# unanan/UNet_Nested4Tiny_Objects_Keypoints

Hardware: AMD Instinct MI355X
Metric: images/sec (train step) UNet++ L=4 256x256 (higher is better)
Workload: dtype f32

## Files before the change

### unet_nested4tiny_objects_keypoints_amd/csrc/gemm_wino.hip

```cpp
#include <cstdlib>
#include <utility>

#include "bn_fused.h"
#include "common.h"
#include "gemm_units.h"
#include "lds_asm.h"
#include "wino_experiments.h"

namespace unetpp {
namespace {

typedef float f32x2 __attribute__((ext_vector_type(2)));
typedef unsigned u32x4v __attribute__((vector_size(16)));
constexpr unsigned kOutOfRange = 0x80000000u;
typedef const __attribute__((address_space(1))) void* gptr_t;
typedef __attribute__((address_space(3))) void* lptr_t;

__device__ __forceinline__ void wino_input_transform(const float (&dd)[16], float (&V)[16]) {
  float t[4][4];
#pragma unroll
  for (int j = 0; j < 4; ++j) {
    t[0][j] = dd[0 + j] - dd[8 + j];
    t[1][j] = dd[4 + j] + dd[8 + j];
    t[2][j] = dd[8 + j] - dd[4 + j];
    t[3][j] = dd[4 + j] - dd[12 + j];
  }
#pragma unroll
  for (int i = 0; i < 4; ++i) {
    V[4 * i + 0] = t[i][0] - t[i][2];
    V[4 * i + 1] = t[i][1] + t[i][2];
    V[4 * i + 2] = t[i][2] - t[i][1];
    V[4 * i + 3] = t[i][1] - t[i][3];
  }
}

__device__ __forceinline__ void wino_input_transform_pk(const f32x2_t (&dd)[8], float (&V)[16]) {
  f32x2_t t[8];
#pragma unroll
  for (int p = 0; p < 2; ++p) {
    t[0 + p] = pk_sub(dd[0 + p], dd[4 + p]);
    t[2 + p] = pk_add(dd[2 + p], dd[4 + p]);
    t[4 + p] = pk_sub(dd[4 + p], dd[2 + p]);
    t[6 + p] = pk_sub(dd[2 + p], dd[6 + p]);
  }
#pragma unroll
  for (int i = 0; i < 4; ++i) {
    const f32x2_t va = pk_sub_add_x(t[2 * i], t[2 * i + 1]);
    const f32x2_t vb = pk_cross_sub(t[2 * i], t[2 * i + 1]);
    V[4 * i + 0] = va[0];
    V[4 * i + 1] = va[1];
    V[4 * i + 2] = vb[0];
    V[4 * i + 3] = vb[1];
  }
}

constexpr int WKC = 8;
constexpr int WNC = 32;
constexpr int WP = 10;
constexpr int WIMG = 4096;

#define WINO_FENCE() __builtin_amdgcn_sched_barrier(0)

template <int LOG2TW, int NH, int MODE, bool BNF = false>
__global__ __launch_bounds__(kThreads, 2) void gemm_wino_kernel(const FastArgs a) {
  constexpr bool LEAN = MODE != 0, FOLD = MODE == 2;
  constexpr int TW = 1 << LOG2TW, TH = kBlockPixels >> LOG2TW;
  constexpr int HWp = TW + 2, HHp = TH + 2;
  constexpr int NPIX = HWp * HHp;
  constexpr int TXN = TW / 2;
  constexpr int IN_FLOATS = 4096;
  constexpr int IN_ITEMS = (NPIX * 2 + kThreads - 1) / kThreads;
  constexpr int W_ITEMS = WIMG / 4 / kThreads;
  static_assert(IN_ITEMS == 3 && W_ITEMS == 4, "the staging lambdas' default ranges");
  static_assert(kMaxHaloPixels * WP <= IN_FLOATS, "input patch does not fit");
  static_assert(((IN_ITEMS * kThreads - 1) >> 1) * WP + 8 <= IN_FLOATS, "staging items past the patch must stay inside the buffer");
  constexpr int BUF = IN_FLOATS + WIMG;
  __shared__ __attribute__((aligned(16))) float smem[2 * BUF];
  float* in_tile = smem;
  float* w_tile = smem + IN_FLOATS;
  constexpr int RUN0 = 4 * WNC * 2;
  __shared__ float stat_lds[BNF ? RUN0 + kBnFusedMaxCols * 2 : RUN0];
  constexpr int kBiasCols = 512;
  __shared__ __attribute__((aligned(16))) float bias_lds[kBiasCols];

  const unetpp_gemm_desc& d = a.d;
  const int tid = threadIdx.x;
  const int wave = __builtin_amdgcn_readfirstlane(tid >> 6), lane = tid & 63, t16 = lane & 15, g = lane >> 4;

  const UnitRange ur = my_contiguous_unit_range(a.total_blocks);
  for (int i = tid; i < kBiasCols; i += kThreads)
    bias_lds[i] = (a.d.bias != nullptr && i < a.Ncols) ? a.d.bias[i] : 0.f;
  constexpr bool bn_fused = BNF;
  if constexpr (BNF) {
    for (int i = tid; i < kBnFusedMaxCols * 2; i += kThreads) stat_lds[RUN0 + i] = 0.f;
  }
  if (ur.count == 0) {
    if constexpr (BNF) {
      __syncthreads();
      bn_rows_store<kThreads>(a.d.stats_partial, a.Ncols, stat_lds + RUN0);
    }
    return;
  }
  const int n_units = __builtin_amdgcn_readfirstlane(static_cast<int>(ur.count));

  const int my_tile = 16 * wave + t16;
  const int a_base = ((2 * (my_tile / TXN)) * HWp + 2 * (my_tile % TXN)) * WP + 2 * g;
  const int b_base = (g * 16 + t16) * 2;

  f32x4 acc[16][NH];
#pragma unroll
  for (int xi = 0; xi < 16; ++xi)
#pragma unroll
    for (int nh = 0; nh < NH; ++nh) acc[xi][nh] = f32x4{0.f, 0.f, 0.f, 0.f};

  f32x4 reg_in[IN_ITEMS];
  unsigned voff[IN_ITEMS];
  unsigned in_mask = 0;
  int pf_cnt = 0;
  int p_unit = 0;
  int p_s = 0, p_c0 = 0, p_chunk = 0;
  int p_n = 0, p_ty0 = 0, p_tx0 = 0;
  const float* p_wimg = nullptr;
  const int cc = (tid & 1) << 2;
  const float* v_ptr = nullptr;
  const float* v_scale = nullptr;
  const float* v_shift = nullptr;
  int v_clen = 0;
  bool v_relu = false;
  int v_bytes = 0, v_pitch = 0, v_origin = 0;
  int pix[IN_ITEMS];
  auto cache_view = [&]() {
    const unetpp_view& V = d.in[p_s];
    v_clen = V.c_len;
    if constexpr (LEAN) {
      v_ptr = V.ptr;
      v_bytes = d.N * V.Hs * V.Ws * V.C * 4;
      v_pitch = V.C * 4;
      v_origin = V.c_off * 4;
      if constexpr (FOLD) {
        v_scale = V.scale;
        v_shift = V.shift;
        v_relu = V.relu != 0;
      }
    } else {
      v_ptr = V.ptr;
      v_scale = V.scale;
      v_shift = V.shift;
      v_relu = V.relu != 0;
    }
  };

  auto step_unit = [&](UnitGeom& u) {
    if (++u.group < a.n_groups) return;
    u.group = 0;
    ++u.patch;
    u.tx0 += TW;
    if (u.tx0 < a.tiles_x * TW) return;
    u.tx0 = 0;
    u.ty0 += TH;
    if (u.ty0 < a.tiles_y * TH) return;
    u.ty0 = 0;
    ++u.n;
  };
  UnitGeom p_ug = decode_unit<LOG2TW>(a, ur.first);
  p_ug.n = __builtin_amdgcn_readfirstlane(p_ug.n);
  p_ug.ty0 = __builtin_amdgcn_readfirstlane(p_ug.ty0);
  p_ug.tx0 = __builtin_amdgcn_readfirstlane(p_ug.tx0);
  p_ug.group = __builtin_amdgcn_readfirstlane(p_ug.group);
  p_ug.patch = __builtin_amdgcn_readfirstlane(static_cast<int>(p_ug.patch));
  UnitGeom c_ug = p_ug;

  long p_patch = -1;
  auto prefetch_unit = [&]() -> bool {
    const UnitGeom& ug = p_ug;
    p_wimg = d.weight_image + static_cast<long>(ug.group) * a.n_chunks * WIMG;
    if (ug.patch == p_patch) return true;
    p_patch = ug.patch;
    p_n = ug.n;
    p_ty0 = ug.ty0;
    p_tx0 = ug.tx0;
    if constexpr (LEAN) {
      const int row0 = p_n * d.H;
#pragma unroll
      for (int q = 0; q < IN_ITEMS; ++q) {
        const int it = tid + q * kThreads;
        const int hp = it >> 1;
        const int hy = hp / HWp, hx = hp - hy * HWp;
        const int y = p_ty0 + hy - 1, x = p_tx0 + hx - 1;
        const bool in_patch = ((q + 1) * kThreads <= NPIX * 2) ? true : (it < NPIX * 2);
        const bool inside = in_patch & (static_cast<unsigned>(y) < static_cast<unsigned>(d.H)) &
                            (static_cast<unsigned>(x) < static_cast<unsigned>(d.W));
        const int linear = (row0 + y) * d.W + x;
        pix[q] = inside ? linear : -1;
      }
      return false;
    }
    in_mask = 0;
#pragma unroll
    for (int q = 0; q < IN_ITEMS; ++q) {
      const int it = tid + q * kThreads;
      const int hp = it >> 1;
      const int hy = hp / HWp, hx = hp - hy * HWp;
      const int y = p_ty0 + hy - 1, x = p_tx0 + hx - 1;
      if ((it < NPIX * 2) && y >= 0 && y < d.H && x >= 0 && x < d.W) in_mask |= 1u << q;
    }
    return false;
  };
  auto view_offsets = [&](const unetpp_view& V) {
    if constexpr (LEAN) {
#pragma unroll
      for (int q = 0; q < IN_ITEMS; ++q)
        voff[q] = static_cast<unsigned>(pix[q] * v_pitch + v_origin + cc * 4) |
                  (static_cast<unsigned>(pix[q] >> 31) & kOutOfRange);
      return;
    }
#pragma unroll
    for (int q = 0; q < IN_ITEMS; ++q) {
      const int hp = min((tid + q * kThreads) >> 1, NPIX - 1);
      const int hy = hp / HWp, hx = hp - hy * HWp;
      const int yy = min(max(p_ty0 + hy - 1, 0), d.H - 1), xx = min(max(p_tx0 + hx - 1, 0), d.W - 1);
      voff[q] = view_pixel_offset32(V, p_n, yy, xx);
    }
  };
  auto advance = [&]() {
    if (p_chunk + 1 < a.n_chunks) {
      ++p_chunk;
      p_c0 += WKC;
      if (p_c0 >= v_clen) {
        ++p_s;
        p_c0 = 0;
        cache_view();
        view_offsets(d.in[p_s]);
      }
    } else if (p_unit + 1 < n_units) {
      ++p_unit;
      p_chunk = 0;
      p_c0 = 0;
      const bool same_view = p_s == 0;
      if (!same_view) {
        p_s = 0;
        cache_view();
      }
      step_unit(p_ug);
      if (!prefetch_unit() || !same_view) view_offsets(d.in[0]);
    }
  };
  f32x4 co_sc = {1.f, 1.f, 1.f, 1.f}, co_sh = {0.f, 0.f, 0.f, 0.f};
  float co_floor = 0.f;
  auto load_coeffs = [&]() {
    if constexpr (!FOLD) return;
    co_floor = v_relu ? 0.f : -__builtin_inff();
    if (v_scale != nullptr) {
      co_sc = *reinterpret_cast<const f32x4*>(v_scale + p_c0 + cc);
      co_sh = *reinterpret_cast<const f32x4*>(v_shift + p_c0 + cc);
    } else {
      co_sc = f32x4{1.f, 1.f, 1.f, 1.f};
      co_sh = f32x4{0.f, 0.f, 0.f, 0.f};
    }
  };
  auto load_inputs = [&]() {
    if constexpr (LEAN) {
      const __amdgpu_buffer_rsrc_t v_rsrc =
          __builtin_amdgcn_make_buffer_rsrc(const_cast<float*>(v_ptr), 0, v_bytes, 0x00020000);
#pragma unroll
      for (int q = 0; q < IN_ITEMS; ++q) {
        const u32x4v v = __builtin_amdgcn_raw_buffer_load_b128(v_rsrc, static_cast<int>(voff[q]), p_c0 * 4, 0);
        reg_in[q] = __builtin_bit_cast(f32x4, v);
      }
      return;
    }
    pf_cnt = min(WKC, v_clen - p_c0);
#pragma unroll
    for (int q = 0; q < IN_ITEMS; ++q) {
      const unsigned off = voff[q] + static_cast<unsigned>(p_c0 + (cc < pf_cnt ? cc : 0));
      reg_in[q] = *reinterpret_cast<const f32x4*>(v_ptr + off);
    }
  };
  auto dma_source = [&]() { return p_wimg + static_cast<long>(p_chunk) * WIMG; };
  auto dma_weights = [&](float* w_dst, const float* wp, int q0 = 0, int q1 = 4) {
#pragma unroll
    for (int q = q0; q < q1; ++q)
      __builtin_amdgcn_global_load_lds((gptr_t)(wp + (tid + q * kThreads) * 4),
                                       (lptr_t)(w_dst + (q * kThreads + wave * 64) * 4), 16, 0, 0);
  };
  auto store_chunk = [&](float* in_dst, int q0 = 0, int q1 = 3) {
    if constexpr (LEAN) {
#pragma unroll
      for (int q = q0; q < q1; ++q) {
        const int it = tid + q * kThreads;
        f32x4 v = reg_in[q];
        if constexpr (FOLD) {
          const unsigned inside = ~static_cast<unsigned>(pix[q] >> 31);
#pragma unroll
          for (int e = 0; e < 4; ++e)
            v[e] = __builtin_bit_cast(float, __builtin_bit_cast(unsigned, floor_keep_nan(fmaf(v[e], co_sc[e], co_sh[e]), co_floor)) & inside);
        }
        *reinterpret_cast<f32x2*>(&in_dst[(it >> 1) * WP + cc]) = f32x2{v[0], v[1]};
        *reinterpret_cast<f32x2*>(&in_dst[(it >> 1) * WP + cc + 2]) = f32x2{v[2], v[3]};
      }
      return;
    }
    const bool affine = v_scale != nullptr;
    f32x4 sc = {1.f, 1.f, 1.f, 1.f}, sh = {0.f, 0.f, 0.f, 0.f};
    if (affine) {
      const int ch = p_c0 + (cc < pf_cnt ? cc : 0);
      sc = *reinterpret_cast<const f32x4*>(v_scale + ch);
      sh = *reinterpret_cast<const f32x4*>(v_shift + ch);
    }
#pragma unroll
    for (int q = 0; q < IN_ITEMS; ++q) {
      const int it = tid + q * kThreads;
      const bool keep = ((in_mask >> q) & 1u) && cc < pf_cnt;
      f32x4 v = reg_in[q];
      if (affine) {
#pragma unroll
        for (int e = 0; e < 4; ++e) v[e] = fmaf(v[e], sc[e], sh[e]);
      }
      if (v_relu) {
#pragma unroll
        for (int e = 0; e < 4; ++e) v[e] = relu_keep_nan(v[e]);
      }
#pragma unroll
      for (int e = 0; e < 4; ++e) v[e] = keep ? v[e] : 0.f;
      if (it < NPIX * 2) {
        *reinterpret_cast<f32x2*>(&in_dst[(it >> 1) * WP + cc]) = f32x2{v[0], v[1]};
        *reinterpret_cast<f32x2*>(&in_dst[(it >> 1) * WP + cc + 2]) = f32x2{v[2], v[3]};
      }
    }
  };

  auto epilogue = [&]() {
    const UnitGeom& ug = c_ug;
    const TileCols tc = decode_tile(a, ug.group);
    const unetpp_view& O = d.out[tc.ov];
    const bool interior = (ug.ty0 + TH <= d.H) && (ug.tx0 + TW <= d.W);
    const unsigned rs = static_cast<unsigned>(O.sy) * O.Ws * O.C, cs = static_cast<unsigned>(O.sx) * O.C;
    const unsigned tile_base = view_pixel_offset32(O, ug.n, ug.ty0, ug.tx0) + tc.nt * WNC;
    float* obase = O.ptr + tile_base;
    const float* gbase = O.gate != nullptr ? O.gate + tile_base : nullptr;
    const bool vec_out = ((O.C | O.c_off | tc.n_cnt) & 3) == 0 && (reinterpret_cast<uintptr_t>(O.ptr) & 15) == 0 &&
                         (O.gate == nullptr || (reinterpret_cast<uintptr_t>(O.gate) & 15) == 0);
    const bool want_stats = d.stats_partial != nullptr;
    const float floor_v = O.relu ? 0.f : -__builtin_inff();
    float s1[NH][4], s2[NH][4];
#pragma unroll
    for (int nh = 0; nh < NH; ++nh)
#pragma unroll
      for (int rr = 0; rr < 4; ++rr) s1[nh][rr] = s2[nh][rr] = 0.f;
    if (d.bias != nullptr && tc.n0 + WNC <= kBiasCols) {
#pragma unroll
      for (int nh = 0; nh < NH; ++nh) acc[5][nh] += *reinterpret_cast<const f32x4*>(&bias_lds[tc.n0 + 16 * nh + 4 * g]);
    } else if (d.bias != nullptr) {
#pragma unroll
      for (int nh = 0; nh < NH; ++nh)
#pragma unroll
        for (int rr = 0; rr < 4; ++rr) {
          const int col = 16 * nh + 4 * g + rr;
          acc[5][nh][rr] += col < tc.n_cnt ? d.bias[tc.n0 + col] : 0.f;
        }
    }
    const unsigned ty2 = 2 * (my_tile / TXN), tx2 = 2 * (my_tile % TXN);
    auto out_row = [&](int ap, int nh, int rr, float (&y)[2]) {
      float tb[4];
#pragma unroll
      for (int b = 0; b < 4; ++b)
        tb[b] = (ap == 0) ? (acc[b][nh][rr] + acc[4 + b][nh][rr]) + acc[8 + b][nh][rr]
                          : (acc[4 + b][nh][rr] - acc[8 + b][nh][rr]) - acc[12 + b][nh][rr];
      y[0] = floor_keep_nan((tb[0] + tb[1]) + tb[2], floor_v);
      y[1] = floor_keep_nan((tb[1] - tb[2]) - tb[3], floor_v);
    };
    if (interior && vec_out && tc.n_cnt == 16 * NH) {
      const bool has_gate = gbase != nullptr, acc_out = O.accumulate != 0;
      const unsigned lane_off = ty2 * rs + tx2 * cs + 4 * g;
#pragma unroll
      for (int ap = 0; ap < 2; ++ap) {
        unsigned off[2][NH];
        f32x4 gt[2][NH], old[2][NH];
#pragma unroll
        for (int bp = 0; bp < 2; ++bp)
#pragma unroll
          for (int nh = 0; nh < NH; ++nh) off[bp][nh] = lane_off + ap * rs + bp * cs + 16 * nh;
        if (has_gate) {
#pragma unroll
          for (int bp = 0; bp < 2; ++bp)
#pragma unroll
            for (int nh = 0; nh < NH; ++nh) gt[bp][nh] = *reinterpret_cast<const f32x4*>(gbase + off[bp][nh]);
        }
        if (acc_out) {
#pragma unroll
          for (int bp = 0; bp < 2; ++bp)
#pragma unroll
            for (int nh = 0; nh < NH; ++nh) old[bp][nh] = *reinterpret_cast<const f32x4*>(obase + off[bp][nh]);
        }
        f32x4 yv[2][NH];
#pragma unroll
        for (int nh = 0; nh < NH; ++nh) {
          f32x2 y[2][2];
#pragma unroll
          for (int cp = 0; cp < 2; ++cp) {
            f32x2 tb[4];
#pragma unroll
            for (int b = 0; b < 4; ++b) {
              const f32x2 m0 = cp ? acc[b][nh].hi : acc[b][nh].lo, m1 = cp ? acc[4 + b][nh].hi : acc[4 + b][nh].lo;
              const f32x2 m2 = cp ? acc[8 + b][nh].hi : acc[8 + b][nh].lo, m3 = cp ? acc[12 + b][nh].hi : acc[12 + b][nh].lo;
              tb[b] = (ap == 0) ? (m0 + m1) + m2 : (m1 - m2) - m3;
            }
            const f32x2 t0 = (tb[0] + tb[1]) + tb[2], t1 = (tb[1] - tb[2]) - tb[3];
            y[0][cp] = f32x2{floor_keep_nan(t0.x, floor_v), floor_keep_nan(t0.y, floor_v)};
            y[1][cp] = f32x2{floor_keep_nan(t1.x, floor_v), floor_keep_nan(t1.y, floor_v)};
          }
          yv[0][nh] = f32x4{y[0][0].x, y[0][0].y, y[0][1].x, y[0][1].y};
          yv[1][nh] = f32x4{y[1][0].x, y[1][0].y, y[1][1].x, y[1][1].y};
          if (want_stats) {
#pragma unroll
            for (int rr = 0; rr < 4; ++rr) {
              const float y0 = yv[0][nh][rr], y1 = yv[1][nh][rr];
              s1[nh][rr] += y0 + y1;
              s2[nh][rr] = fmaf(y0, y0, fmaf(y1, y1, s2[nh][rr]));
            }
          }
        }
        if (!has_gate && !acc_out) {
#pragma unroll
          for (int bp = 0; bp < 2; ++bp)
#pragma unroll
            for (int nh = 0; nh < NH; ++nh) {
              if constexpr (wino_exp::kNoOutStore) asm volatile("" ::"v"(yv[bp][nh]), "v"(off[bp][nh]));
              else *reinterpret_cast<f32x4*>(obase + off[bp][nh]) = yv[bp][nh];
            }
          continue;
        }
#pragma unroll
        for (int bp = 0; bp < 2; ++bp)
#pragma unroll
          for (int nh = 0; nh < NH; ++nh) {
            f32x4 v = yv[bp][nh];
            if (has_gate && !O.gate_sum) {
#pragma unroll
              for (int e = 0; e < 4; ++e) v[e] = (gt[bp][nh][e] > 0.f) ? v[e] : 0.f;
            }
            if (acc_out) {
#pragma unroll
              for (int e = 0; e < 4; ++e) v[e] += old[bp][nh][e];
            }
            if (has_gate && O.gate_sum) {
#pragma unroll
              for (int e = 0; e < 4; ++e) v[e] = (gt[bp][nh][e] > 0.f) ? v[e] : 0.f;
            }
            *reinterpret_cast<f32x4*>(obase + off[bp][nh]) = v;
          }
      }
    } else {
#pragma unroll
      for (int ap = 0; ap < 2; ++ap) {
        const unsigned py = ty2 + ap;
#pragma unroll
        for (int nh = 0; nh < NH; ++nh)
#pragma unroll
          for (int rr = 0; rr < 4; ++rr) {
            float y[2];
            out_row(ap, nh, rr, y);
            const int col = 16 * nh + 4 * g + rr;
#pragma unroll
            for (int bp = 0; bp < 2; ++bp) {
              float v = y[bp];
              if ((col < tc.n_cnt) && (ug.ty0 + py < d.H) && (ug.tx0 + tx2 + bp < d.W)) {
                s1[nh][rr] += v;
                s2[nh][rr] = fmaf(v, v, s2[nh][rr]);
                const unsigned off = py * rs + (tx2 + bp) * cs + col;
                if (gbase != nullptr && !O.gate_sum) v = (gbase[off] > 0.f) ? v : 0.f;
                if (O.accumulate) v += obase[off];
                if (gbase != nullptr && O.gate_sum) v = (gbase[off] > 0.f) ? v : 0.f;
                obase[off] = v;
              }
            }
          }
      }
    }
#pragma unroll
    for (int xi = 0; xi < 16; ++xi)
#pragma unroll
      for (int nh = 0; nh < NH; ++nh) acc[xi][nh] = f32x4{0.f, 0.f, 0.f, 0.f};
    if (want_stats) {
#pragma unroll
      for (int nh = 0; nh < NH; ++nh)
#pragma unroll
        for (int rr = 0; rr < 4; ++rr) {
          s1[nh][rr] = row16_sum(s1[nh][rr]);
          s2[nh][rr] = row16_sum(s2[nh][rr]);
          if (t16 == 0) {
            stat_lds[(wave * WNC + 16 * nh + 4 * g + rr) * 2 + 0] = s1[nh][rr];
            stat_lds[(wave * WNC + 16 * nh + 4 * g + rr) * 2 + 1] = s2[nh][rr];
          }
        }
    }
  };
  auto flush_stats = [&]() {
    if (d.stats_partial == nullptr || tid >= 16 * NH) return;
    const UnitGeom& ug = c_ug;
    const TileCols tc = decode_tile(a, ug.group);
    if (tid >= tc.n_cnt) return;
    float t1 = 0.f, t2 = 0.f;
#pragma unroll
    for (int w = 0; w < 4; ++w) {
      t1 += stat_lds[(w * WNC + tid) * 2 + 0];
      t2 += stat_lds[(w * WNC + tid) * 2 + 1];
    }
    if constexpr (bn_fused) {
      stat_lds[RUN0 + (tc.n0 + tid) * 2 + 0] += t1;
      stat_lds[RUN0 + (tc.n0 + tid) * 2 + 1] += t2;
      return;
    }
    float* dst = d.stats_partial + (ug.patch * a.Ncols + tc.n0 + tid) * 2;
    dst[0] = t1;
    dst[1] = t2;
  };

  cache_view();
  prefetch_unit();
  view_offsets(d.in[0]);
  load_coeffs();
  load_inputs();
  dma_weights(w_tile, dma_source());
  store_chunk(in_tile);
  advance();
  load_coeffs();
  load_inputs();
  asm volatile("s_waitcnt vmcnt(%0)" ::"n"(IN_ITEMS) : "memory");
  __syncthreads();

  int c_chunk = 0, c_unit = 0;
  int cur = 0;
  while (true) {
    const unsigned in_b = lds_offset(in_tile) + a_base * 4, w_b = lds_offset(w_tile) + b_base * 4;
    float dd[16], ddn[16], V[16];
    f32x2_t dp[8], dpn[8];
    unsigned row_b[4];
#pragma unroll
    for (int i = 0; i < 4; ++i) row_b[i] = in_b + i * HWp * WP * 4;
    f32x4 us[2][2];
    if constexpr (LEAN) {
      static_for<8>([&](auto ic) {
        constexpr int e = decltype(ic)::v, j = 2 * (e & 1);
        lds_read2_b32<j * WP, (j + 1) * WP>(dp[e], row_b[e >> 1]);
      });
    } else {
      static_for<16>([&](auto ic) {
        constexpr int e = decltype(ic)::v;
        lds_read_b32<((e / 4) * HWp + (e % 4)) * WP * 4>(dd[e], in_b);
      });
    }
    lds_read2st64_b64<0, 1>(us[0][0], w_b);
    lds_read2st64_b64<2, 3>(us[0][1], w_b);

    float* other = smem + (cur ^ 1) * BUF;
    if constexpr (!LEAN) {
      __builtin_amdgcn_s_setprio(3);
      store_chunk(other);
      dma_weights(other + IN_FLOATS, dma_source());
      advance();
      load_inputs();
    }
    auto staging_piece = [&](auto gc) {
      constexpr int g = decltype(gc)::v;
      if constexpr (!LEAN) return;
      if constexpr (wino_exp::kNoStaging) {
        if constexpr (g == 2) advance();
        return;
      }
      if constexpr (g == 0 && !wino_exp::kNoStore) store_chunk(other);
      if constexpr (g == 0 && !wino_exp::kNoDma) dma_weights(other + IN_FLOATS, dma_source());
      if constexpr (g == 1) {
        advance();
        load_coeffs();
      }
      if constexpr (g == 2 && !wino_exp::kNoLoads) load_inputs();
    };

    __builtin_amdgcn_s_setprio(2);
    if constexpr (LEAN) {
      lds_wait8x2(dp);
      lds_wait(us[0][0], us[0][1]);
      wino_input_transform_pk(dp, V);
    } else {
      lds_wait16(dd);
      lds_wait(us[0][0], us[0][1]);
      wino_input_transform(dd, V);
    }
    static_for<8>([&](auto gc) {
      constexpr int g = decltype(gc)::v, cs = g & 1, ns = cs ^ 1;
      if constexpr (g + 1 < 8) {
        lds_read2st64_b64<4 * (g + 1), 4 * (g + 1) + 1>(us[ns][0], w_b);
        lds_read2st64_b64<4 * (g + 1) + 2, 4 * (g + 1) + 3>(us[ns][1], w_b);
      }
      if constexpr (g == 0) {
        if constexpr (LEAN) {
          static_for<8>([&](auto ic) {
            constexpr int e = decltype(ic)::v, j = 2 * (e & 1);
            lds_read2_b32<j * WP + 1, (j + 1) * WP + 1>(dpn[e], row_b[e >> 1]);
          });
        } else {
          static_for<16>([&](auto ic) {
            constexpr int e = decltype(ic)::v;
            lds_read_b32<(((e / 4) * HWp + (e % 4)) * WP + 1) * 4>(ddn[e], in_b);
          });
        }
      }
      WINO_FENCE();
#pragma unroll
      for (int q = 0; q < 4; ++q) {
        const int xi = (4 * g + q) & 15;
        const f32x4 up = us[cs][q >> 1];
        acc[xi][0] = __builtin_amdgcn_mfma_f32_16x16x4f32(up[(q & 1) * 2], V[xi], acc[xi][0], 0, 0, 0);
        if (NH == 2)
          acc[xi][NH - 1] = __builtin_amdgcn_mfma_f32_16x16x4f32(up[(q & 1) * 2 + 1], V[xi], acc[xi][NH - 1], 0, 0, 0);
      }
      staging_piece(gc);
      WINO_FENCE();
      if constexpr (g == 0) {
        if constexpr (LEAN) lds_wait8x2(dpn);
        else lds_wait16(ddn);
      }
      if constexpr (g + 1 < 8) lds_wait(us[ns][0], us[ns][1]);
      if constexpr (g == 3) {
        if constexpr (LEAN) wino_input_transform_pk(dpn, V);
        else wino_input_transform(ddn, V);
      }
    });
    __builtin_amdgcn_s_setprio(0);
    if constexpr (!wino_exp::kNoBarrier) {
      if (wino_exp::kLaxWait && c_chunk == 0 && c_unit > 0)
        asm volatile("s_waitcnt vmcnt(%0) lgkmcnt(0)" ::"n"(IN_ITEMS + 4 + 4 * NH) : "memory");
      else
      asm volatile("s_waitcnt vmcnt(%0) lgkmcnt(0)" ::"n"(IN_ITEMS) : "memory");
      __builtin_amdgcn_s_barrier();
      asm volatile("" ::: "memory");
    }
    if (c_chunk + 1 == a.n_chunks) {
#pragma unroll
      for (int q = 0; q < IN_ITEMS; ++q) asm volatile("" : "+v"(reg_in[q]));
      if constexpr (wino_exp::kNoEpilogue) {
#pragma unroll
        for (int xi = 0; xi < 16; ++xi)
#pragma unroll
          for (int nh = 0; nh < NH; ++nh) {
            asm volatile("" : "+v"(acc[xi][nh]));
            acc[xi][nh] = f32x4{0.f, 0.f, 0.f, 0.f};
          }
      } else {
        epilogue();
      }
      if (d.stats_partial != nullptr) {
        __syncthreads();
        flush_stats();
      }
      step_unit(c_ug);
      c_chunk = 0;
      if (++c_unit == n_units) break;
    } else {
      ++c_chunk;
    }
    cur ^= 1;
    in_tile = smem + cur * BUF;
    w_tile = in_tile + IN_FLOATS;
  }
  if constexpr (BNF) {
    __syncthreads();
    bn_rows_store<kThreads>(d.stats_partial, a.Ncols, stat_lds + RUN0);
  }
}

}

bool wino_applies(const unetpp_gemm_desc* d) {
  return d != nullptr && d->taps == 9 && (d->flags & (UNETPP_GEMM_DIRECT | UNETPP_GEMM_BF16)) == 0;
}

void gemm_wino_plan(const unetpp_gemm_desc* d, GemmSel& s) {
  s.kernel = GEMM_WINO;
  s.label = "gemm_wino_kernel";
  long workers = (2L * s.cus) & ~7L;
#ifdef UNETPP_WINO_EXP
  if (opt_value(OPT_WINO_ONE_PER_CU, 0) == 1) workers = s.cus & ~7L;
#endif
  if (workers < 8) workers = 8;
  if (workers > kBnFusedRows) workers = kBnFusedRows;
  s.grid_x = static_cast<unsigned>(s.fa.total_blocks <= workers ? s.fa.total_blocks : workers);
  bool narrow = true;
  for (int i = 0; i < d->n_out; ++i) narrow = narrow && d->out[i].c_len <= 16;
  bool lean = opt_value(OPT_WINO_NO_LEAN, 0) == 0, fold = false;
  for (int i = 0; i < d->n_in; ++i) {
    const unetpp_view& v = d->in[i];
    lean = lean && (v.c_len & 7) == 0 && v.Hs == d->H && v.Ws == d->W && v.sy == 1 && v.sx == 1 && v.oy == 0 &&
           v.ox == 0 && static_cast<long>(d->N) * v.Hs * v.Ws * v.C * 4 <= 0x7fffffffL;
    fold = fold || v.scale != nullptr || v.relu != 0;
  }
  s.narrow = narrow ? 1 : 0;
  s.mode = !lean ? 0 : (fold ? 2 : 1);
  s.fa.bn_in_kernel = (s.mode != 0 && bn_rows_per_workgroup(d, s.fa.Ncols)) ? 1 : 0;
  s.bn_rows = s.fa.bn_in_kernel ? s.grid_x : 0;
}

int launch_gemm_wino(const unetpp_gemm_desc*, const GemmSel& s, hipStream_t st) {
  const FastArgs& a = s.fa;
  const int mode = s.mode;
  const bool narrow = s.narrow != 0;
  const dim3 grid(s.grid_x), block(kThreads);
#define UNETPP_LAUNCH_WINO_M(L, NHV)                                                                    \
  do {                                                                                                  \
    if (mode == 0) hipLaunchKernelGGL((gemm_wino_kernel<L, NHV, 0>), grid, block, 0, st, a);            \
    else if (a.bn_in_kernel && mode == 1) hipLaunchKernelGGL((gemm_wino_kernel<L, NHV, 1, true>), grid, block, 0, st, a); \
    else if (a.bn_in_kernel) hipLaunchKernelGGL((gemm_wino_kernel<L, NHV, 2, true>), grid, block, 0, st, a);             \
    else if (mode == 1) hipLaunchKernelGGL((gemm_wino_kernel<L, NHV, 1>), grid, block, 0, st, a);       \
    else hipLaunchKernelGGL((gemm_wino_kernel<L, NHV, 2>), grid, block, 0, st, a);                      \
  } while (0)
#define UNETPP_LAUNCH_WINO(L)                 \
  do {                                        \
    if (narrow) UNETPP_LAUNCH_WINO_M(L, 1);   \
    else UNETPP_LAUNCH_WINO_M(L, 2);          \
  } while (0)
  if (a.log2tw == 5) UNETPP_LAUNCH_WINO(5);
  else if (a.log2tw == 4) UNETPP_LAUNCH_WINO(4);
  else UNETPP_LAUNCH_WINO(3);
#undef UNETPP_LAUNCH_WINO
#undef UNETPP_LAUNCH_WINO_M
  return launch_status();
}

}
```

### unet_nested4tiny_objects_keypoints_amd/csrc/lds_asm.h

```cpp
#pragma once
#include <utility>

#include "common.h"

namespace unetpp {

template <int I>
struct IC {
  static constexpr int v = I;
};
template <class F, int... I>
__device__ __forceinline__ void static_for_impl(F&& f, std::integer_sequence<int, I...>) {
  (f(IC<I>{}), ...);
}
template <int N, class F>
__device__ __forceinline__ void static_for(F&& f) {
  static_for_impl(f, std::make_integer_sequence<int, N>{});
}
__device__ __forceinline__ unsigned lds_offset(const float* p) {
  return static_cast<unsigned>(reinterpret_cast<uintptr_t>(p));
}
template <int OFF>
__device__ __forceinline__ void lds_read_b32(float& v, unsigned addr) {
  asm volatile("ds_read_b32 %0, %1 offset:%2" : "=v"(v) : "v"(addr), "n"(OFF));
}
template <int O0, int O1>
__device__ __forceinline__ void lds_read2st64_b64(f32x4& v, unsigned addr) {
  asm volatile("ds_read2st64_b64 %0, %1 offset0:%2 offset1:%3" : "=v"(v) : "v"(addr), "n"(O0), "n"(O1));
}
typedef float f32x2_t __attribute__((ext_vector_type(2)));
template <int O0, int O1>
__device__ __forceinline__ void lds_read2_b32(f32x2_t& v, unsigned addr) {
  asm volatile("ds_read2_b32 %0, %1 offset0:%2 offset1:%3" : "=v"(v) : "v"(addr), "n"(O0), "n"(O1));
}
__device__ __forceinline__ void lds_wait8x2(f32x2_t (&d)[8]) {
  asm volatile("s_waitcnt lgkmcnt(0)"
               : "+v"(d[0]), "+v"(d[1]), "+v"(d[2]), "+v"(d[3]), "+v"(d[4]), "+v"(d[5]), "+v"(d[6]), "+v"(d[7]));
}
__device__ __forceinline__ void lds_wait4x2(f32x2_t (&d)[4]) {
  asm volatile("s_waitcnt lgkmcnt(0)" : "+v"(d[0]), "+v"(d[1]), "+v"(d[2]), "+v"(d[3]));
}
__device__ __forceinline__ f32x2_t pk_add(f32x2_t a, f32x2_t b) {
  f32x2_t r;
  asm("v_pk_add_f32 %0, %1, %2" : "=v"(r) : "v"(a), "v"(b));
  return r;
}
__device__ __forceinline__ f32x2_t pk_sub(f32x2_t a, f32x2_t b) {
  f32x2_t r;
  asm("v_pk_add_f32 %0, %1, %2 neg_lo:[0,1] neg_hi:[0,1]" : "=v"(r) : "v"(a), "v"(b));
  return r;
}
__device__ __forceinline__ f32x2_t pk_sub_add_x(f32x2_t a, f32x2_t b) {
  f32x2_t r;
  asm("v_pk_add_f32 %0, %1, %2 op_sel:[0,0] op_sel_hi:[1,0] neg_lo:[0,1] neg_hi:[0,0]" : "=v"(r) : "v"(a), "v"(b));
  return r;
}
__device__ __forceinline__ f32x2_t pk_cross_sub(f32x2_t a, f32x2_t b) {
  f32x2_t r;
  asm("v_pk_add_f32 %0, %1, %2 op_sel:[0,1] op_sel_hi:[1,1] neg_lo:[0,1] neg_hi:[1,0]" : "=v"(r) : "v"(b), "v"(a));
  return r;
}
__device__ __forceinline__ f32x2_t pk_sum_diff(f32x2_t a) {
  f32x2_t r;
  asm("v_pk_add_f32 %0, %1, %1 op_sel:[0,1] op_sel_hi:[0,1] neg_lo:[0,0] neg_hi:[0,1]" : "=v"(r) : "v"(a));
  return r;
}
__device__ __forceinline__ void lds_wait(f32x4& a, f32x4& b) {
  asm volatile("s_waitcnt lgkmcnt(0)" : "+v"(a), "+v"(b));
}
__device__ __forceinline__ void lds_wait4(float (&d)[4]) {
  asm volatile("s_waitcnt lgkmcnt(0)" : "+v"(d[0]), "+v"(d[1]), "+v"(d[2]), "+v"(d[3]));
}
__device__ __forceinline__ void lds_wait16(float (&d)[16]) {
  asm volatile("s_waitcnt lgkmcnt(0)"
               : "+v"(d[0]), "+v"(d[1]), "+v"(d[2]), "+v"(d[3]), "+v"(d[4]), "+v"(d[5]), "+v"(d[6]), "+v"(d[7]));
  asm volatile("s_waitcnt lgkmcnt(0)"
               : "+v"(d[8]), "+v"(d[9]), "+v"(d[10]), "+v"(d[11]), "+v"(d[12]), "+v"(d[13]), "+v"(d[14]), "+v"(d[15]));
}

}
```

### unet_nested4tiny_objects_keypoints_amd/csrc/weight_image.hip

```cpp
#include "bf16_common.h"
#include "common.h"
#include "gemm_units.h"

namespace unetpp {
namespace {


struct PackGeom {
  int kind, taps, kc, ncol;
  int n_in, n_out;
  int in_len[UNETPP_MAX_VIEWS], out_len[UNETPP_MAX_VIEWS];
  int n_chunks, n_tiles;
  long floats;
};

__host__ __device__ inline long image_floats_per_tile_chunk(int kind, int taps) { return kind == kKindWino ? 4096 : taps * 512L; }

__host__ __device__ inline void finish_geom(PackGeom& g) {
  g.n_chunks = 0;
  g.n_tiles = 0;
  for (int i = 0; i < g.n_in; ++i) g.n_chunks += (g.in_len[i] + g.kc - 1) / g.kc;
  for (int i = 0; i < g.n_out; ++i) g.n_tiles += (g.out_len[i] + g.ncol - 1) / g.ncol;
  g.floats = static_cast<long>(g.n_tiles) * g.n_chunks * image_floats_per_tile_chunk(g.kind, g.taps);
}

__device__ __forceinline__ float wsrc_at(const unetpp_weight_src& w, int taps, int tap, int k, int n) {
  const int tt = w.flip ? taps - 1 - tap : tap;
  const int ki = w.k_inner > 0 ? k % w.k_inner : k, ko = w.k_inner > 0 ? k / w.k_inner : 0;
  const int ni = w.n_inner > 0 ? n % w.n_inner : n, no = w.n_inner > 0 ? n / w.n_inner : 0;
  return w.src[tt * w.s_t + ki * w.s_k + ko * w.s_ko + ni * w.s_n + no * w.s_no];
}

struct RowOrigin {
  int k0, k_room;
  int n0, n_room;
};
__device__ __forceinline__ RowOrigin row_origin(const PackGeom& g, int nt, int chunk) {
  int kbase = 0, v = 0;
  for (; v < g.n_in - 1; ++v) {
    const int ch = (g.in_len[v] + g.kc - 1) / g.kc;
    if (chunk < ch) break;
    chunk -= ch;
    kbase += g.in_len[v];
  }
  int col_base = 0, ov = 0;
  for (; ov < g.n_out - 1; ++ov) {
    const int tv = (g.out_len[ov] + g.ncol - 1) / g.ncol;
    if (nt < tv) break;
    nt -= tv;
    col_base += g.out_len[ov];
  }
  RowOrigin o;
  o.k0 = kbase + chunk * g.kc;
  o.k_room = g.in_len[v] - chunk * g.kc;
  o.n0 = col_base + nt * g.ncol;
  o.n_room = g.out_len[ov] - nt * g.ncol;
  return o;
}

__device__ __forceinline__ void fill_image_row(const PackGeom& g, const unetpp_weight_src& w, long row, float* __restrict__ img) {
  const int tid = threadIdx.x;
  if (g.kind == kKindWino) {
    const RowOrigin o = row_origin(g, static_cast<int>(row / g.n_chunks), static_cast<int>(row % g.n_chunks));
    const int t = tid;
    const int kk = 2 * ((t >> 5) & 3) + ((t >> 7) & 1), cl = 16 * (t & 1) + ((t >> 1) & 15);
    float* dst = img + row * 4096 + (t & 127) + (static_cast<long>(t >> 7) << 11);
    if (kk >= o.k_room || cl >= o.n_room) {
#pragma unroll
      for (int xi = 0; xi < 16; ++xi) dst[xi << 7] = 0.f;
      return;
    }
    const int k = o.k0 + kk, n = o.n0 + cl;
    float tr[4][3];
#pragma unroll
    for (int c = 0; c < 3; ++c) {
      const float w0 = wsrc_at(w, 9, 0 * 3 + c, k, n), w1 = wsrc_at(w, 9, 1 * 3 + c, k, n), w2 = wsrc_at(w, 9, 2 * 3 + c, k, n);
      tr[0][c] = w0;
      tr[1][c] = 0.5f * (w0 + w1 + w2);
      tr[2][c] = 0.5f * (w0 - w1 + w2);
      tr[3][c] = w2;
    }
#pragma unroll
    for (int ra = 0; ra < 4; ++ra) {
      dst[(4 * ra + 0) << 7] = tr[ra][0];
      dst[(4 * ra + 1) << 7] = 0.5f * (tr[ra][0] + tr[ra][1] + tr[ra][2]);
      dst[(4 * ra + 2) << 7] = 0.5f * (tr[ra][0] - tr[ra][1] + tr[ra][2]);
      dst[(4 * ra + 3) << 7] = tr[ra][2];
    }
    return;
  }
  const int tap = static_cast<int>(row % g.taps);
  const long rc = row / g.taps;
  const RowOrigin o = row_origin(g, static_cast<int>(rc / g.n_chunks), static_cast<int>(rc % g.n_chunks));
  float* dst = img + row * 512;
#pragma unroll
  for (int q = 0; q < 2; ++q) {
    const int e = tid + q * 256;
    if (g.kind == kKindBf16) {
      const int i0 = 2 * e;
      const int kk = 16 * ((i0 >> 9) & 1) + 8 * ((i0 >> 3) & 1) + (i0 & 7), cl = (i0 >> 4) & 31;
      float a = 0.f, b = 0.f;
      if (cl < o.n_room) {
        if (kk < o.k_room) a = wsrc_at(w, g.taps, tap, o.k0 + kk, o.n0 + cl);
        if (kk + 1 < o.k_room) b = wsrc_at(w, g.taps, tap, o.k0 + kk + 1, o.n0 + cl);
      }
      dst[e] = __uint_as_float(pack_bf2(a, b));
    } else {
      const int j = (e >> 3) & 31;
      const int kk = 8 * ((e >> 8) & 1) + 4 * (((e >> 2) & 1) ^ ((j >> 3) & 1)) + (e & 3);
      dst[e] = (kk < o.k_room && j < o.n_room) ? wsrc_at(w, g.taps, tap, o.k0 + kk, o.n0 + j) : 0.f;
    }
  }
}

__device__ __forceinline__ void fill_bf16_3x3_block(const PackGeom& g, const unetpp_weight_src& w, long rc,
                                                     float* __restrict__ img, float* lds ) {
  const int tid = threadIdx.x;
  const RowOrigin o = row_origin(g, static_cast<int>(rc / g.n_chunks), static_cast<int>(rc % g.n_chunks));
  const bool k_inner_most = w.s_k < w.s_n;
  __syncthreads();
  const long inner_stride = k_inner_most ? w.s_k : w.s_n, outer_stride = k_inner_most ? w.s_n : w.s_k;
  const int inner_room = k_inner_most ? o.k_room : o.n_room, outer_room = k_inner_most ? o.n_room : o.k_room;
  const long origin = static_cast<long>(o.k0) * w.s_k + static_cast<long>(o.n0) * w.s_n;
  const bool wide = w.s_t == 1 && inner_stride == 9 && w.k_inner <= 0 && w.n_inner <= 0 && inner_room >= 32 &&
                    ((reinterpret_cast<uintptr_t>(w.src + origin) | static_cast<uintptr_t>(outer_stride * 4)) & 15) == 0;
  if (wide) {
#pragma unroll 3
    for (int q = tid; q < 32 * 72; q += 256) {
      const int oo = q / 72, r4 = q - oo * 72;
      f32x4 v = {0.f, 0.f, 0.f, 0.f};
      if (oo < outer_room) v = *reinterpret_cast<const f32x4*>(w.src + origin + oo * outer_stride + 4 * r4);
#pragma unroll
      for (int c = 0; c < 4; ++c) {
        const int f = 4 * r4 + c, m = f / 9;
        const int tap_m = f - 9 * m, tap = w.flip ? 8 - tap_m : tap_m;
        const int kk = k_inner_most ? m : oo, cl = k_inner_most ? oo : m;
        lds[(tap * 32 + kk) * 33 + cl] = v[c];
      }
    }
  } else {
#pragma unroll 6
    for (int idx = tid; idx < 9 * 32 * 32; idx += 256) {
      const int tap = idx % 9, m = (idx / 9) & 31, oo = idx / (9 * 32);
      const int kk = k_inner_most ? m : oo, cl = k_inner_most ? oo : m;
      lds[(tap * 32 + kk) * 33 + cl] = (kk < o.k_room && cl < o.n_room) ? wsrc_at(w, 9, tap, o.k0 + kk, o.n0 + cl) : 0.f;
    }
  }
  __syncthreads();
  f32x4* dst4 = reinterpret_cast<f32x4*>(img + rc * 9 * 512);
#pragma unroll 3
  for (int s4 = tid; s4 < 9 * 128; s4 += 256) {
    const int tap = s4 >> 7, e4 = s4 & 127;
    const int cl = (e4 >> 1) & 31, kk0 = 16 * ((e4 >> 6) & 1) + 8 * (e4 & 1);
    f32x4 out;
#pragma unroll
    for (int c = 0; c < 4; ++c)
      out[c] = __uint_as_float(pack_bf2(lds[(tap * 32 + kk0 + 2 * c) * 33 + cl], lds[(tap * 32 + kk0 + 2 * c + 1) * 33 + cl]));
    dst4[s4] = out;
  }
}

__device__ __forceinline__ float image_element(const PackGeom& g, const unetpp_weight_src& w, long i) {
  int kk, cin_local, tap = 0, xi = 0;
  long r;
  if (g.kind == kKindWino) {
    const int nh = i & 1, col = (i >> 1) & 15, gq = (i >> 5) & 3, s = (i >> 11) & 1;
    xi = (i >> 7) & 15;
    kk = 2 * gq + s;
    cin_local = 16 * nh + col;
    r = i >> 12;
  } else if (g.kind == kKindBf16) {
    const int e = i & 7, hs = (i >> 3) & 1, j = (i >> 4) & 31, gq = (i >> 9) & 1;
    r = i >> 10;
    tap = static_cast<int>(r % g.taps);
    r /= g.taps;
    kk = 16 * gq + 8 * hs + e;
    cin_local = j;
  } else {
    const int e = i & 3, hs = (i >> 2) & 1, j = (i >> 3) & 31, gq = (i >> 8) & 1;
    r = i >> 9;
    tap = static_cast<int>(r % g.taps);
    r /= g.taps;
    kk = 8 * gq + 4 * (hs ^ ((j >> 3) & 1)) + e;
    cin_local = j;
  }
  int chunk = static_cast<int>(r % g.n_chunks);
  int nt = static_cast<int>(r / g.n_chunks);
  int kbase = 0, v = 0;
  for (; v < g.n_in - 1; ++v) {
    const int ch = (g.in_len[v] + g.kc - 1) / g.kc;
    if (chunk < ch) break;
    chunk -= ch;
    kbase += g.in_len[v];
  }
  const int kin = chunk * g.kc + kk;
  int col_base = 0, ov = 0;
  for (; ov < g.n_out - 1; ++ov) {
    const int tv = (g.out_len[ov] + g.ncol - 1) / g.ncol;
    if (nt < tv) break;
    nt -= tv;
    col_base += g.out_len[ov];
  }
  const int cin = nt * g.ncol + cin_local;
  if (kin >= g.in_len[v] || cin >= g.out_len[ov]) return 0.f;
  const int k = kbase + kin, n = col_base + cin;
  if (g.kind != kKindWino) return wsrc_at(w, g.taps, tap, k, n);
  const int ra = xi >> 2, rb = xi & 3;
  float t[3];
#pragma unroll
  for (int c = 0; c < 3; ++c) {
    const float w0 = wsrc_at(w, 9, 0 * 3 + c, k, n), w1 = wsrc_at(w, 9, 1 * 3 + c, k, n), w2 = wsrc_at(w, 9, 2 * 3 + c, k, n);
    t[c] = ra == 0 ? w0 : (ra == 1 ? 0.5f * (w0 + w1 + w2) : (ra == 2 ? 0.5f * (w0 - w1 + w2) : w2));
  }
  return rb == 0 ? t[0] : (rb == 1 ? 0.5f * (t[0] + t[1] + t[2]) : (rb == 2 ? 0.5f * (t[0] - t[1] + t[2]) : t[2]));
}

__device__ __forceinline__ float image_slot(const PackGeom& g, const unetpp_weight_src& w, long i) {
  if (g.kind != kKindBf16) return image_element(g, w, i);
  return __uint_as_float(pack_bf2(image_element(g, w, 2 * i), image_element(g, w, 2 * i + 1)));
}

__global__ void pack_image_one_kernel(const PackGeom g, const unetpp_weight_src w, float* __restrict__ img) {
  const long i = blockIdx.x * static_cast<long>(blockDim.x) + threadIdx.x;
  if (i < g.floats) img[i] = image_slot(g, w, i);
}

__global__ void pack_image_jobs_kernel(const unetpp_pack_job* __restrict__ jobs) {
  const unetpp_pack_job& j = jobs[blockIdx.y];
  __shared__ PackGeom g;
  if (threadIdx.x == 0) {
    const bool bf = (j.flags & UNETPP_GEMM_BF16) != 0;
    const bool wino = !bf && j.taps == 9 && (j.flags & UNETPP_GEMM_DIRECT) == 0;
    g.kind = bf ? kKindBf16 : (wino ? kKindWino : kKindFast);
    g.taps = j.taps;
    g.kc = bf ? 32 : (wino ? 8 : 16);
    g.ncol = 32;
    g.n_in = j.n_in;
    g.n_out = j.n_out;
    for (int i = 0; i < UNETPP_MAX_VIEWS; ++i) {
      g.in_len[i] = j.in_len[i];
      g.out_len[i] = j.out_len[i];
    }
    finish_geom(g);
  }
  __syncthreads();
  if (g.kind == kKindBf16 && g.taps == 9) {
    __shared__ float stage[9 * 32 * 33];
    const long blocks = g.floats / (9 * 512);
    for (long rc = blockIdx.x; rc < blocks; rc += gridDim.x) fill_bf16_3x3_block(g, j.src, rc, j.image, stage);
    return;
  }
  const long rows = g.floats / (g.kind == kKindWino ? 4096 : 512);
  for (long row = blockIdx.x; row < rows; row += gridDim.x) fill_image_row(g, j.src, row, j.image);
}

bool geom_of(const unetpp_gemm_desc* d, PackGeom& g) {
  GemmSel s;
  if (!gemm_image_of(d, s)) return false;
  g.kind = s.image_kind;
  g.taps = d->taps;
  g.kc = s.image_kc;
  g.ncol = 32;
  g.n_in = d->n_in;
  g.n_out = d->n_out;
  for (int i = 0; i < UNETPP_MAX_VIEWS; ++i) {
    g.in_len[i] = i < d->n_in ? d->in[i].c_len : 0;
    g.out_len[i] = i < d->n_out ? d->out[i].c_len : 0;
  }
  g.n_chunks = s.fa.n_chunks;
  g.n_tiles = s.fa.n_tiles;
  g.floats = s.image_floats;
  return true;
}

}
}

using namespace unetpp;

extern "C" int64_t unetpp_gemm_weight_image_floats(const unetpp_gemm_desc* d) {
  PackGeom g;
  return geom_of(d, g) ? g.floats : 0;
}

extern "C" int unetpp_gemm_pack_weight_image_from(const unetpp_gemm_desc* d, const unetpp_weight_src* src, float* image,
                                                  void* stream) {
  PackGeom g;
  if (src == nullptr || src->src == nullptr || image == nullptr || !geom_of(d, g)) return UNETPP_EINVAL;
  hipLaunchKernelGGL(pack_image_one_kernel, dim3(static_cast<unsigned>((g.floats + 255) / 256)), dim3(256), 0,
                     static_cast<hipStream_t>(stream), g, *src, image);
  return launch_status();
}

extern "C" int unetpp_gemm_pack_weight_image(const unetpp_gemm_desc* d, float* image, void* stream) {
  if (d == nullptr || d->weight == nullptr) return UNETPP_EINVAL;
  long K = 0, N = 0;
  for (int i = 0; i < d->n_in && i < UNETPP_MAX_VIEWS; ++i) K += d->in[i].c_len;
  for (int i = 0; i < d->n_out && i < UNETPP_MAX_VIEWS; ++i) N += d->out[i].c_len;
  unetpp_weight_src w = {};
  w.src = d->weight;
  w.s_t = K * N;
  w.s_k = N;
  w.s_n = 1;
  return unetpp_gemm_pack_weight_image_from(d, &w, image, stream);
}

extern "C" int unetpp_gemm_pack_weight_images(const unetpp_pack_job* jobs_device, int32_t n_jobs, int64_t max_image_floats,
                                              void* stream) {
  if (jobs_device == nullptr || n_jobs < 1 || n_jobs > 65535 || max_image_floats < 1) return UNETPP_EINVAL;
  long bx = (max_image_floats + 256L * 8 - 1) / (256L * 8);
  if (bx > 256) bx = 256;
  hipLaunchKernelGGL(pack_image_jobs_kernel, dim3(static_cast<unsigned>(bx), static_cast<unsigned>(n_jobs)), dim3(256), 0,
                     static_cast<hipStream_t>(stream), jobs_device);
  return launch_status();
}
```

Before: 1731.

## Use planar LDS input layout and b128 weight reads in Winograd kernel

The LEAN Winograd path now stores the staged input patch in a channel-planar LDS layout with a stride of 400 floats per plane. Window rows can then be fetched with single ds_read_b64 instead of paired ds_read2_b32. The packed weight image is reordered so each lane's weights are contiguous, which lets ds_read_b128 replace ds_read2st64_b64. The NaN-preserving floor is also swapped for a plain maximum, which cuts instructions but may change NaN propagation.

```diff
diff --git a/unet_nested4tiny_objects_keypoints_amd/csrc/gemm_wino.hip b/unet_nested4tiny_objects_keypoints_amd/csrc/gemm_wino.hip
--- a/unet_nested4tiny_objects_keypoints_amd/csrc/gemm_wino.hip
+++ b/unet_nested4tiny_objects_keypoints_amd/csrc/gemm_wino.hip
@@ -58,6 +58,9 @@
 constexpr int WNC = 32;
 constexpr int WP = 10;
 constexpr int WIMG = 4096;
+constexpr int WPL = 400;
+
+__device__ __forceinline__ float floor_max(float v, float floor_v) { return __builtin_elementwise_maximum(v, floor_v); }
 
 #define WINO_FENCE() __builtin_amdgcn_sched_barrier(0)
 
@@ -74,6 +77,9 @@
   static_assert(IN_ITEMS == 3 && W_ITEMS == 4, "the staging lambdas' default ranges");
   static_assert(kMaxHaloPixels * WP <= IN_FLOATS, "input patch does not fit");
   static_assert(((IN_ITEMS * kThreads - 1) >> 1) * WP + 8 <= IN_FLOATS, "staging items past the patch must stay inside the buffer");
+  static_assert(WKC * WPL <= IN_FLOATS && NPIX <= WPL, "planar input patch does not fit");
+  static_assert(((IN_ITEMS * kThreads - 1) >> 1) < WPL, "staging items past the patch must stay inside their own plane");
+  static_assert((2 * WPL) % 64 == 32 && WPL % 2 == 0 && HWp % 2 == 0, "conflict-free, 8-byte aligned ds_read_b64 of the window rows");
   constexpr int BUF = IN_FLOATS + WIMG;
   __shared__ __attribute__((aligned(16))) float smem[2 * BUF];
   float* in_tile = smem;
@@ -104,8 +110,9 @@
   const int n_units = __builtin_amdgcn_readfirstlane(static_cast<int>(ur.count));
 
   const int my_tile = 16 * wave + t16;
-  const int a_base = ((2 * (my_tile / TXN)) * HWp + 2 * (my_tile % TXN)) * WP + 2 * g;
-  const int b_base = (g * 16 + t16) * 2;
+  const int a_pixel = (2 * (my_tile / TXN)) * HWp + 2 * (my_tile % TXN);
+  const int a_base = LEAN ? 2 * g * WPL + a_pixel : a_pixel * WP + 2 * g;
+  const int b_base = (g * 16 + t16) * 4;
 
   f32x4 acc[16][NH];
 #pragma unroll
@@ -293,10 +300,10 @@
           const unsigned inside = ~static_cast<unsigned>(pix[q] >> 31);
 #pragma unroll
           for (int e = 0; e < 4; ++e)
-            v[e] = __builtin_bit_cast(float, __builtin_bit_cast(unsigned, floor_keep_nan(fmaf(v[e], co_sc[e], co_sh[e]), co_floor)) & inside);
+            v[e] = __builtin_bit_cast(float, __builtin_bit_cast(unsigned, floor_max(fmaf(v[e], co_sc[e], co_sh[e]), co_floor)) & inside);
         }
-        *reinterpret_cast<f32x2*>(&in_dst[(it >> 1) * WP + cc]) = f32x2{v[0], v[1]};
-        *reinterpret_cast<f32x2*>(&in_dst[(it >> 1) * WP + cc + 2]) = f32x2{v[2], v[3]};
+#pragma unroll
+        for (int e = 0; e < 4; ++e) in_dst[(cc + e) * WPL + (it >> 1)] = v[e];
       }
       return;
     }
@@ -366,8 +373,8 @@
       for (int b = 0; b < 4; ++b)
         tb[b] = (ap == 0) ? (acc[b][nh][rr] + acc[4 + b][nh][rr]) + acc[8 + b][nh][rr]
                           : (acc[4 + b][nh][rr] - acc[8 + b][nh][rr]) - acc[12 + b][nh][rr];
-      y[0] = floor_keep_nan((tb[0] + tb[1]) + tb[2], floor_v);
-      y[1] = floor_keep_nan((tb[1] - tb[2]) - tb[3], floor_v);
+      y[0] = floor_max((tb[0] + tb[1]) + tb[2], floor_v);
+      y[1] = floor_max((tb[1] - tb[2]) - tb[3], floor_v);
     };
     if (interior && vec_out && tc.n_cnt == 16 * NH) {
       const bool has_gate = gbase != nullptr, acc_out = O.accumulate != 0;
@@ -406,8 +413,8 @@
               tb[b] = (ap == 0) ? (m0 + m1) + m2 : (m1 - m2) - m3;
             }
             const f32x2 t0 = (tb[0] + tb[1]) + tb[2], t1 = (tb[1] - tb[2]) - tb[3];
-            y[0][cp] = f32x2{floor_keep_nan(t0.x, floor_v), floor_keep_nan(t0.y, floor_v)};
-            y[1][cp] = f32x2{floor_keep_nan(t1.x, floor_v), floor_keep_nan(t1.y, floor_v)};
+            y[0][cp] = f32x2{floor_max(t0.x, floor_v), floor_max(t0.y, floor_v)};
+            y[1][cp] = f32x2{floor_max(t1.x, floor_v), floor_max(t1.y, floor_v)};
           }
           yv[0][nh] = f32x4{y[0][0].x, y[0][0].y, y[0][1].x, y[0][1].y};
           yv[1][nh] = f32x4{y[1][0].x, y[1][0].y, y[1][1].x, y[1][1].y};
@@ -535,14 +542,11 @@
     const unsigned in_b = lds_offset(in_tile) + a_base * 4, w_b = lds_offset(w_tile) + b_base * 4;
     float dd[16], ddn[16], V[16];
     f32x2_t dp[8], dpn[8];
-    unsigned row_b[4];
-#pragma unroll
-    for (int i = 0; i < 4; ++i) row_b[i] = in_b + i * HWp * WP * 4;
     f32x4 us[2][2];
     if constexpr (LEAN) {
       static_for<8>([&](auto ic) {
-        constexpr int e = decltype(ic)::v, j = 2 * (e & 1);
-        lds_read2_b32<j * WP, (j + 1) * WP>(dp[e], row_b[e >> 1]);
+        constexpr int e = decltype(ic)::v;
+        lds_read_b64<((e >> 1) * HWp + 2 * (e & 1)) * 4>(dp[e], in_b);
       });
     } else {
       static_for<16>([&](auto ic) {
@@ -550,8 +554,8 @@
         lds_read_b32<((e / 4) * HWp + (e % 4)) * WP * 4>(dd[e], in_b);
       });
     }
-    lds_read2st64_b64<0, 1>(us[0][0], w_b);
-    lds_read2st64_b64<2, 3>(us[0][1], w_b);
+    lds_read_b128<0>(us[0][0], w_b);
+    lds_read_b128<1024>(us[0][1], w_b);
 
     float* other = smem + (cur ^ 1) * BUF;
     if constexpr (!LEAN) {
@@ -590,14 +594,14 @@
     static_for<8>([&](auto gc) {
       constexpr int g = decltype(gc)::v, cs = g & 1, ns = cs ^ 1;
       if constexpr (g + 1 < 8) {
-        lds_read2st64_b64<4 * (g + 1), 4 * (g + 1) + 1>(us[ns][0], w_b);
-        lds_read2st64_b64<4 * (g + 1) + 2, 4 * (g + 1) + 3>(us[ns][1], w_b);
+        lds_read_b128<2048 * (g + 1)>(us[ns][0], w_b);
+        lds_read_b128<2048 * (g + 1) + 1024>(us[ns][1], w_b);
       }
       if constexpr (g == 0) {
         if constexpr (LEAN) {
           static_for<8>([&](auto ic) {
-            constexpr int e = decltype(ic)::v, j = 2 * (e & 1);
-            lds_read2_b32<j * WP + 1, (j + 1) * WP + 1>(dpn[e], row_b[e >> 1]);
+            constexpr int e = decltype(ic)::v;
+            lds_read_b64<(WPL + (e >> 1) * HWp + 2 * (e & 1)) * 4>(dpn[e], in_b);
           });
         } else {
           static_for<16>([&](auto ic) {
diff --git a/unet_nested4tiny_objects_keypoints_amd/csrc/lds_asm.h b/unet_nested4tiny_objects_keypoints_amd/csrc/lds_asm.h
--- a/unet_nested4tiny_objects_keypoints_amd/csrc/lds_asm.h
+++ b/unet_nested4tiny_objects_keypoints_amd/csrc/lds_asm.h
@@ -24,11 +24,15 @@
 __device__ __forceinline__ void lds_read_b32(float& v, unsigned addr) {
   asm volatile("ds_read_b32 %0, %1 offset:%2" : "=v"(v) : "v"(addr), "n"(OFF));
 }
-template <int O0, int O1>
-__device__ __forceinline__ void lds_read2st64_b64(f32x4& v, unsigned addr) {
-  asm volatile("ds_read2st64_b64 %0, %1 offset0:%2 offset1:%3" : "=v"(v) : "v"(addr), "n"(O0), "n"(O1));
+template <int OFF>
+__device__ __forceinline__ void lds_read_b128(f32x4& v, unsigned addr) {
+  asm volatile("ds_read_b128 %0, %1 offset:%2" : "=v"(v) : "v"(addr), "n"(OFF));
 }
 typedef float f32x2_t __attribute__((ext_vector_type(2)));
+template <int OFF>
+__device__ __forceinline__ void lds_read_b64(f32x2_t& v, unsigned addr) {
+  asm volatile("ds_read_b64 %0, %1 offset:%2" : "=v"(v) : "v"(addr), "n"(OFF));
+}
 template <int O0, int O1>
 __device__ __forceinline__ void lds_read2_b32(f32x2_t& v, unsigned addr) {
   asm volatile("ds_read2_b32 %0, %1 offset0:%2 offset1:%3" : "=v"(v) : "v"(addr), "n"(O0), "n"(O1));
diff --git a/unet_nested4tiny_objects_keypoints_amd/csrc/weight_image.hip b/unet_nested4tiny_objects_keypoints_amd/csrc/weight_image.hip
--- a/unet_nested4tiny_objects_keypoints_amd/csrc/weight_image.hip
+++ b/unet_nested4tiny_objects_keypoints_amd/csrc/weight_image.hip
@@ -64,10 +64,11 @@
     const RowOrigin o = row_origin(g, static_cast<int>(row / g.n_chunks), static_cast<int>(row % g.n_chunks));
     const int t = tid;
     const int kk = 2 * ((t >> 5) & 3) + ((t >> 7) & 1), cl = 16 * (t & 1) + ((t >> 1) & 15);
-    float* dst = img + row * 4096 + (t & 127) + (static_cast<long>(t >> 7) << 11);
+    float* dst = img + row * 4096 + (t & 1) + (((t >> 1) & 63) << 2) + (static_cast<long>(t >> 7) << 11);
+    auto slot = [](int xi) { return ((xi & 1) << 1) + ((xi >> 1) << 8); };
     if (kk >= o.k_room || cl >= o.n_room) {
 #pragma unroll
-      for (int xi = 0; xi < 16; ++xi) dst[xi << 7] = 0.f;
+      for (int xi = 0; xi < 16; ++xi) dst[slot(xi)] = 0.f;
       return;
     }
     const int k = o.k0 + kk, n = o.n0 + cl;
@@ -82,10 +83,10 @@
     }
 #pragma unroll
     for (int ra = 0; ra < 4; ++ra) {
-      dst[(4 * ra + 0) << 7] = tr[ra][0];
-      dst[(4 * ra + 1) << 7] = 0.5f * (tr[ra][0] + tr[ra][1] + tr[ra][2]);
-      dst[(4 * ra + 2) << 7] = 0.5f * (tr[ra][0] - tr[ra][1] + tr[ra][2]);
-      dst[(4 * ra + 3) << 7] = tr[ra][2];
+      dst[slot(4 * ra + 0)] = tr[ra][0];
+      dst[slot(4 * ra + 1)] = 0.5f * (tr[ra][0] + tr[ra][1] + tr[ra][2]);
+      dst[slot(4 * ra + 2)] = 0.5f * (tr[ra][0] - tr[ra][1] + tr[ra][2]);
+      dst[slot(4 * ra + 3)] = tr[ra][2];
     }
     return;
   }
@@ -164,8 +165,8 @@
   int kk, cin_local, tap = 0, xi = 0;
   long r;
   if (g.kind == kKindWino) {
-    const int nh = i & 1, col = (i >> 1) & 15, gq = (i >> 5) & 3, s = (i >> 11) & 1;
-    xi = (i >> 7) & 15;
+    const int nh = i & 1, col = (i >> 2) & 15, gq = (i >> 6) & 3, s = (i >> 11) & 1;
+    xi = (((i >> 8) & 7) << 1) | ((i >> 1) & 1);
     kk = 2 * gq + s;
     cin_local = 16 * nh + col;
     r = i >> 12;
```

Measured after the change: 1763 (median of 6 runs). 1.02x the previous value.
